# scale-lab/MTLoRA

Hardware: AMD Instinct MI355X
Metric: images/sec (train step) Swin-T/448 r=64 4-task (higher is better)
Workload: dtype bf16; 1 GPU; BASELINE configs[1]: Swin-T 448, 4 tasks (semseg,normals,sal,human_parts), r_shared=64 r_task=4 scale4; train step (fwd+loss+bwd+clip+AdamW), dropout .05, drop_path .2; per_gpu_batch=32, global_batch=32, img_size=448, parallelism=dp1, trainable_params=8344634, allreduce_bytes=0

## Files before the change

mtlora_amd/csrc/linear.hip:

```cpp
#include <string.h>
#include <algorithm>
#include <atomic>
#include <type_traits>

#include "common.h"
#include "internal.h"
#include "hid_params.h"
#include "nt.h"
#include "stream.h"
#include "dense.h"
#include "pq.h"
#include "tn.h"

namespace {

static Segs make_segs(const mtlora_linear_desc* d) {
    Segs s;
    s.n = 1 + d->T;
    int off = 0;
    for (int o = 0; o < s.n; ++o) {
        int r = (o == 0) ? d->r_s : d->r_t[o - 1];
        s.r[o] = r;
        s.rp[o] = (int)mtl_round_up(r, 8);
        s.off[o] = off;
        off += s.rp[o];
    }
    for (int o = s.n; o < MAXO; ++o) s.r[o] = s.rp[o] = s.off[o] = 0;
    s.used = off;
    s.R = (int)mtl_round_up(off, 16);
    return s;
}

static CtxLayout ctx_layout(const mtlora_linear_desc* d, const Segs& s) {
    const int es = mtl_elem_size(d->dtype);
    CtxLayout L;
    int64_t o = 0;
    auto take = [&](int64_t bytes) {
        int64_t at = o;
        o += mtl_round_up(bytes, 256);
        return at;
    };
    L.a_cat = take((int64_t)s.R * d->K * es);
    L.b_cat = take((int64_t)d->N * s.R * es);
    L.at_cat = take((int64_t)d->K * s.R * es);
    L.bt_cat = take((int64_t)s.R * d->N * es);
    L.alpha = take((int64_t)s.R * 4);
    L.a_proj = take((int64_t)s.R * d->K * es);
    L.bt_proj = take((int64_t)s.R * d->N * es);
    L.b_frag = take(mtl_round_up(d->N, 32) * mtl_round_up(s.R, 32) * es);
    L.at_frag = take(mtl_round_up(d->K, 32) * mtl_round_up(s.R, 32) * es);
    L.pack_total = o;
    if (d->packed) o = 0;
    L.p = take(d->M * s.R * es);
    L.total = o;
    return L;
}

static int check_desc(const mtlora_linear_desc* d) {
    if (!d) return MTLORA_ERR_NULL;
    if (d->dtype != MTLORA_F32 && d->dtype != MTLORA_BF16 && d->dtype != MTLORA_F16) return MTLORA_ERR_DTYPE;
    if (d->M < 0 || d->K <= 0 || d->N <= 0 || d->T < 0 || d->T > MTLORA_MAX_TASKS || d->r_s < 0)
        return MTLORA_ERR_SHAPE;
    if (d->M >= ((int64_t)1 << 31)) return MTLORA_ERR_SHAPE;
    const int vec = d->dtype == MTLORA_F32 ? 4 : 8;
    if (d->K % vec || d->N % vec) return MTLORA_ERR_ALIGN;
    for (int t = 0; t < d->T; ++t)
        if (d->r_t[t] <= 0) return MTLORA_ERR_SHAPE;
    if (d->mode != 0 && d->mode != 1) return MTLORA_ERR_UNSUPPORTED;
    if (d->bwd_phase < 0 || d->bwd_phase > 2) return MTLORA_ERR_UNSUPPORTED;
    if (d->sel_stream < 0 || d->sel_stream > 1 || d->sel_dense < 0 || d->sel_dense > 4 || d->sel_tn < 0 || d->sel_tn > 2 || d->sel_projk < 0 ||
        d->sel_projk > 3 || d->max_cu < 0)
        return MTLORA_ERR_UNSUPPORTED;
    if (d->dropout_p < 0.f || d->dropout_p >= 1.f) return MTLORA_ERR_SHAPE;
    return MTLORA_OK;
}

static bool misaligned(const void* p) { return ((uintptr_t)p & 15u) != 0; }

struct Tune {
    int sp, ntd, tn, projk, max_cu;
};
static Tune make_tune(const mtlora_linear_desc* d) {
    auto tri = [](int v) { return v == 1 ? 0 : (v == 2 ? 2 : 1); };
    Tune t;
    t.sp = d->sel_stream == 1 ? 0 : 1;
    t.ntd = d->sel_dense >= 3 ? d->sel_dense : tri(d->sel_dense);
    t.tn = tri(d->sel_tn);
    t.projk = d->sel_projk == 3 ? 3 : tri(d->sel_projk);
    t.max_cu = d->max_cu > 0 ? d->max_cu : 0;
    return t;
}
constexpr int MTL_MAX_DEV = 64;
static int cur_dev() {
    int dev = 0;
    (void)hipGetDevice(&dev);
    return dev >= 0 && dev < MTL_MAX_DEV ? dev : 0;
}
static int dev_num_cu() {
    static std::atomic<int> cache[MTL_MAX_DEV];
    const int dev = cur_dev();
    int cu = cache[dev].load(std::memory_order_relaxed);
    if (cu == 0) {
        cu = 256;
        (void)hipDeviceGetAttribute(&cu, hipDeviceAttributeMultiprocessorCount, dev);
        if (cu <= 0) cu = 256;
        cache[dev].store(cu, std::memory_order_relaxed);
    }
    return cu;
}
static int num_cu(const Tune& tu) {
    const int cu = dev_num_cu();
    return tu.max_cu > 0 && tu.max_cu < cu ? tu.max_cu : cu;
}
static bool raise_lds(std::atomic<unsigned long long>& done, const void* fn, int bytes) {
    const int dev = cur_dev();
    if ((done.load(std::memory_order_relaxed) >> dev) & 1ull) return true;
    if (hipFuncSetAttribute(fn, hipFuncAttributeMaxDynamicSharedMemorySize, bytes) != hipSuccess) {
        (void)hipGetLastError();
        return false;
    }
    done.fetch_or(1ull << dev, std::memory_order_relaxed);
    return true;
}
#define MTL_RAISE_LDS(KERNEL, BYTES)                                        \
    do {                                                                    \
        static std::atomic<unsigned long long> done__{0};                   \
        (void)raise_lds(done__, (const void*)(KERNEL), (int)(BYTES));       \
    } while (0)

static bool nte_prefer(int64_t tiles, int ksteps, int64_t cus) {
    const double eff_d = (double)tiles / (double)(mtl_ceil_div(tiles, cus) * cus);
    return (ksteps >= 4 && ksteps <= 12 && tiles * 2 >= 3 * cus) || (ksteps >= 6 && eff_d < 0.7 && tiles >= cus);
}

static NlParams make_nl(const NtParams& P, int64_t mt, int64_t nt, bool dense) {
    NlParams q;
    q.act = reinterpret_cast<const bf16*>(P.act[0]);
    q.wgt = reinterpret_cast<const bf16*>(P.wgt);
    q.L = reinterpret_cast<const bf16*>(P.L);
    q.Rm = reinterpret_cast<const bf16*>(P.Rm);
    q.out = reinterpret_cast<bf16*>(P.out[0].ptr);
    q.act2 = reinterpret_cast<bf16*>(P.out[0].act);
    q.gate = dense ? reinterpret_cast<const bf16*>(P.out[0].gate) : nullptr;
    q.bias = P.bias;
    q.alpha = P.alpha;
    q.ld_act = P.ld_act;
    q.ld_wgt = P.ld_wgt;
    q.ldL = P.ldL;
    q.ldR = P.ldR;
    q.ld_out = P.ld_out;
    q.M = (int)P.M;
    q.n_rows = P.n_rows;
    q.K = P.act[0] ? P.K : 0;
    q.seg_lo = P.L ? P.out[0].seg_lo : 0;
    q.seg_hi = P.L ? P.out[0].seg_hi : 0;
    q.n_tiles = (int)nt;
    q.nt_magic = (uint32_t)(((uint64_t)1 << 32) / (uint64_t)nt) + 1u;
    const uint32_t nwg = (uint32_t)(mt * nt);
    q.q8 = nwg / 8u;
    q.r8 = nwg % 8u;
    q.act_mask = dense ? 0 : P.act_mask;
    q.use_base = P.out[0].use_base;
    q.drop = P.drop;
    return q;
}

template <typename F>
static void nl_dispatch(const NlParams& q, bool ml0, F&& go) {
    using Y = std::true_type;
// ... 162 lines not shown
    MtlProfScope prof(kind, alg_bytes, s, s8d, flops);
    const size_t lds = (size_t)q.n_blk_total * 32 * q.K * 2 + (size_t)SP_WAVES * ns * 32 * ch * 2;
    const int per_cu = lds * 2 <= (size_t)SP_LDS_MAX ? 2 : 1;
    int64_t wgs = mtl_ceil_div(q.n_items, SP_WAVES);
    if (wgs > (int64_t)num_cu(tu) * per_cu) wgs = (int64_t)num_cu(tu) * per_cu;
#define MTL_SP_PROJ(CHV, NSV)                                                                              \
    do {                                                                                                   \
        MTL_RAISE_LDS((k_sp_proj<T, CHV, NSV>), SP_LDS_MAX);                                               \
        hipLaunchKernelGGL((k_sp_proj<T, CHV, NSV>), dim3((unsigned)wgs), dim3(64 * SP_WAVES), lds, s, q); \
    } while (0)
    if constexpr (sizeof(T) == 2) {
        if (ch == 96) {
            if (ns == 3) MTL_SP_PROJ(96, 3);
            else if (ns == 2) MTL_SP_PROJ(96, 2);
            else MTL_SP_PROJ(96, 1);
        } else {
            if (ns == 3) MTL_SP_PROJ(64, 3);
            else if (ns == 2) MTL_SP_PROJ(64, 2);
            else MTL_SP_PROJ(64, 1);
        }
    }
#undef MTL_SP_PROJ
}

template <typename T>
static int pq_plan(const Tune& tu, const SpProjParams& q, PqParams& pq) {
    if (sizeof(T) != 2 || tu.sp == 0 || tu.projk == 0 || tu.projk == 2 || q.M <= 0 || q.n_src < 1 || q.n_src > MAXO) return 0;
    if (q.Rw % 8 != 0 || q.K % 8 != 0 || q.K < 32 || (q.ld_out % 8) != 0) return 0;
    if ((((uintptr_t)q.wproj | (uintptr_t)q.out) & 15u) != 0) return 0;
    if (q.M >= ((int64_t)1 << 31) - 256 || q.M * q.ld_out * 2 >= ((int64_t)1 << 32) - 64) return 0;
    int wmax = 0;
    for (int s = 0; s < q.n_src; ++s) {
        const SpSrc& ss = q.src[s];
        if (((uintptr_t)ss.act & 15u) != 0 || ss.col_lo % 8 != 0 || ss.col_hi % 8 != 0 || ss.col_hi <= ss.col_lo || ss.col_hi > q.Rw) return 0;
        if (ss.col_hi - ss.col_lo > 1024) return 0;
        pq.src[s].act = ss.act;
        pq.src[s].col_lo = ss.col_lo;
        pq.src[s].col_hi = ss.col_hi;
        pq.src[s].mask = ss.mask;
        pq.src[s].pad_ = 0;
        wmax = ss.col_hi - ss.col_lo > wmax ? ss.col_hi - ss.col_lo : wmax;
    }
    pq.n_src = q.n_src;
    pq.wproj = q.wproj;
    pq.out = q.out;
    pq.ld_out = q.ld_out;
    pq.M = (int)q.M;
    pq.K = q.K;
    pq.R = q.Rw;
    pq.drop = q.drop;
    const int64_t per_row_tile = (int64_t)q.n_src * mtl_ceil_div(wmax, wmax > 64 ? 128 : 64);
    return mtl_ceil_div(q.M, 64) * per_row_tile * 4 <= (int64_t)num_cu(tu) * 5 ? 1 : 2;
}
static bool pq_one_round(const Tune& tu, const PqParams& pq, int mb) {
    return pq.n_src == 1 && mtl_ceil_div(pq.M, 64 * mb) * 4 <= (int64_t)num_cu(tu) * 5;
}
template <typename T>
static void launch_pq(const PqParams& pq, int mb, hipStream_t s, int kind, double alg_bytes, double s8d, double flops) {
    int wmax = 0, any_mask = 0;
    for (int i = 0; i < pq.n_src; ++i) {
        wmax = pq.src[i].col_hi - pq.src[i].col_lo > wmax ? pq.src[i].col_hi - pq.src[i].col_lo : wmax;
        any_mask |= pq.src[i].mask;
    }
    mtl_prof_tag("pq M%d K%d R%d src%d w%d mb%d mask%d", pq.M, pq.K, pq.R, pq.n_src, wmax, mb, any_mask);
    MtlProfScope prof(kind, alg_bytes, s, s8d, flops);
    const bool wide = wmax > 64;
    const dim3 grid((unsigned)mtl_ceil_div(pq.M, 64 * mb), (unsigned)mtl_ceil_div(wmax, wide ? 128 : 64), (unsigned)pq.n_src);
#define MTL_PQ(WMV, NBV, NSTV, KSV)                                                                               \
    do {                                                                                                          \
        constexpr size_t lds = (size_t)NSTV * (32 * WMV + 32 * NBV) * 64;                                         \
        MTL_RAISE_LDS((k_pq<T, WMV, NBV, NSTV, KSV>), SP_LDS_MAX);                                                \
        hipLaunchKernelGGL((k_pq<T, WMV, NBV, NSTV, KSV>), grid, dim3(256), lds, s, pq);                          \
    } while (0)
    if constexpr (sizeof(T) == 2) {
        const bool ksp = any_mask != 0 && pq.drop.enabled();
        if (mb == 1 && wide && ksp) MTL_PQ(2, 4, 6, true);
        else if (mb == 1 && wide) MTL_PQ(2, 4, 6, false);
        else if (mb == 1 && ksp) MTL_PQ(2, 2, 8, true);
        else if (mb == 1) MTL_PQ(2, 2, 8, false);
        else if (wide) MTL_PQ(4, 4, 5, false);
        else MTL_PQ(4, 2, 6, false);
    }
#undef MTL_PQ
}

template <typename T>
static bool sp_projk_plan(const Tune& tu, SpProjParams& q, int& ch) {
    if (sizeof(T) != 2 || tu.sp == 0 || q.M <= 0 || q.n_src <= 0) return false;
    const int mode = tu.projk;
    if (mode == 0) return false;
    ch = q.K % 96 == 0 ? 96 : (q.K % 64 == 0 ? 64 : 0);
    if (ch == 0 || q.M >= ((int64_t)1 << 31) - 64) return false;
    q.n_blk_total = (q.Rw + 31) / 32;
    for (int s = 0; s < q.n_src; ++s) {
        if (q.src[s].n_blk > SP_MAXB || q.src[s].n_blk <= 0) return false;
        if (((uintptr_t)q.src[s].act & 15u) != 0) return false;
    }
    if ((q.ld_out % 8) != 0 || ((uintptr_t)q.out & 15u) != 0 || ((uintptr_t)q.wproj & 15u) != 0) return false;
    if (q.M * q.ld_out * 2 >= ((int64_t)1 << 32) - 64) return false;
    q.n_slabs = (int)mtl_ceil_div(q.M, 32);
    q.n_items = q.n_slabs * q.n_src;
    return mode == 2 || (mode == 1 && (int64_t)q.n_items <= (int64_t)num_cu(tu) && q.K / ch >= SP_WAVES);
}
template <typename T>
static void launch_sp_projk(const Tune& tu, const SpProjParams& q, int ch, hipStream_t s, int kind, double alg_bytes, double s8d, double flops) {
    mtl_prof_tag("sp_projk M%lld K%d R%d src%d ch%d", (long long)q.M, q.K, q.Rw, q.n_src, ch);
    MtlProfScope prof(kind, alg_bytes, s, s8d, flops);
    int64_t wgs = q.n_items;
    if (wgs > (int64_t)num_cu(tu)) wgs = num_cu(tu);
#define MTL_SP_PROJK(CHV, NSLV)                                                                                   \
    do {                                                                                                          \
        constexpr size_t slots = (size_t)SP_WAVES * NSLV * 32 * CHV * 2, red = (size_t)SP_WAVES * SP_MAXB * 4096; \
        constexpr size_t lds = slots > red ? slots : red;                                                         \
        MTL_RAISE_LDS((k_sp_projk<T, CHV, NSLV>), SP_LDS_MAX);                                                    \
        hipLaunchKernelGGL((k_sp_projk<T, CHV, NSLV>), dim3((unsigned)wgs), dim3(64 * SP_WAVES), lds, s, q);      \
    } while (0)
    if constexpr (sizeof(T) == 2) {
        if (ch == 96)
            MTL_SP_PROJK(96, 3);
        else
            MTL_SP_PROJK(64, 4);
    }
#undef MTL_SP_PROJK
}

template <typename T>
static void launch_sp_projsum(const Tune& tu, const SpProjParams& q, int ch, int ns, T* gsum, hipStream_t s, int kind, double alg_bytes,
                              double s8d, double flops) {
    mtl_prof_tag("sp_projsum M%lld K%d R%d src%d ch%d ns%d", (long long)q.M, q.K, q.Rw, q.n_src, ch, ns);
    MtlProfScope prof(kind, alg_bytes, s, s8d, flops);
    const size_t lds = (size_t)q.n_blk_total * 32 * q.K * 2 + (size_t)SP_WAVES * ns * 32 * ch * 2;
    int64_t wgs = mtl_ceil_div(q.n_slabs, SP_WAVES);
    if (wgs > (int64_t)num_cu(tu)) wgs = num_cu(tu);
#define MTL_SP_PS(CHV, NSV)                                                                                         \
    do {                                                                                                            \
        MTL_RAISE_LDS((k_sp_projsum<T, CHV, NSV>), SP_LDS_MAX);                                                     \
        hipLaunchKernelGGL((k_sp_projsum<T, CHV, NSV>), dim3((unsigned)wgs), dim3(64 * SP_WAVES), lds, s, q, gsum); \
    } while (0)
    if constexpr (sizeof(T) == 2) {
        if (ch == 96) {
            if (ns >= 2) MTL_SP_PS(96, 2);
            else MTL_SP_PS(96, 1);
        } else {
            if (ns >= 2) MTL_SP_PS(64, 2);
            else MTL_SP_PS(64, 1);
        }
    }
#undef MTL_SP_PS
}

struct SpXresPlan {
    int ch, nkc, nrb;
    bool stg;
    unsigned grid;
    size_t lds;
};
static unsigned sp_lin_grid(const Tune& tu, int parts, int n_slabs, int& xsh) {
    const int64_t cu = num_cu(tu);
    const int64_t by_slabs = mtl_ceil_div(n_slabs, SP_WAVES);
    if (cu >= 8 * (int64_t)parts) {
        xsh = 3;
        int64_t g8 = mtl_ceil_div(by_slabs, 8);
        const int64_t g8_max = cu / (8 * parts);
        if (g8 > g8_max) g8 = g8_max;
        return (unsigned)(8 * parts * g8);
    }
// ... 399 lines not shown
        q.drop = dc;
        if (j.one_panel) {
            q.act[0] = src[0].act;
            q.act_mask = src[0].mask;
            q.n_rows = sg.R;
        } else {
            for (int i = 0; i < n_src; ++i) {
                q.zact[i] = src[i].act;
                q.zrow0[i] = src[i].col_lo;
                q.zrows[i] = src[i].col_hi - src[i].col_lo;
                q.zmask[i] = src[i].mask;
            }
            q.nz = n_src;
        }
        launch_nt<T>(tu, q, s, j.kind, j.alg_bytes, j.s8d, j.flops);
    }
}

static double rank_sum(const Segs& sg, const void* const* live = nullptr) {
    double rsum = 0.0;
    for (int o = 0; o < sg.n; ++o)
        if (!live || (sg.rp[o] > 0 && live[o])) rsum += sg.r[o];
    return rsum;
}
static double fused_bytes(const mtlora_linear_desc* d, int es) { return (double)es * d->M * (d->K + (double)d->N); }
static double fused_flops(const mtlora_linear_desc* d, const Segs& sg) {
    return 2.0 * d->M * (double)d->K * d->N + 2.0 * d->M * (double)sg.r[0] * (d->K + d->N);
}

template <typename T>
static bool fwd_one_pass(const mtlora_linear_desc* d, const Tune& tu, const Segs& sg, const CtxLayout& L, const unsigned char* pk, const void* x,
                         const void* W, const float* bias, void* y_s, void* a_s, T* Pm, const DropoutCfg& dc, hipStream_t s) {
    SpLinParams q = {};
    q.act = x;
    q.w = W;
    q.proj = pk + L.a_proj;
    q.expand = pk + L.b_frag;
    q.bias = bias;
    q.out = y_s;
    q.out2 = a_s;
    q.pout = Pm;
    q.ld_out = d->N;
    q.ldp = sg.R;
    q.M = d->M;
    q.n_cols = (int)d->N;
    q.R = sg.R;
    q.mask_act = 1;
    q.mask_lr = 0;
    q.drop = dc;
    SpXresPlan pl;
    const double b8d = fused_bytes(d, (int)sizeof(T)), fl = fused_flops(d, sg);
    if (sp_xres_plan<T>(tu, q, (int)d->K, pl)) {
        launch_sp_xres<T>(q, pl, a_s != nullptr, s, PK_NT_FWD_MAIN, b8d + (a_s ? (double)sizeof(T) * d->M * d->N : 0.0), b8d, fl);
        return true;
    }
    SpAresPlan pa;
    q.estep = q.estep2 = 0;
    if (a_s == nullptr && sp_ares_plan<T>(tu, q, (int)d->K, pa)) {
        launch_sp_ares<T>(q, pa, s, PK_NT_FWD_MAIN, b8d, b8d, fl);
        return true;
    }
    return false;
}

template <typename T>
static int fwd_impl(const mtlora_linear_desc* d, const void* x, const void* const* x_t, const void* W,
                    const float* bias, const float* A_s, const float* B_s, const float* const* A_t,
                    const float* const* B_t, void* y_s, void* const* y_t, void* ctx, hipStream_t s, void* a_s = nullptr,
                    void* const* a_t = nullptr) {
    const Segs sg = make_segs(d);
    const Tune tu = make_tune(d);
    const CtxLayout L = ctx_layout(d, sg);
    unsigned char* c = reinterpret_cast<unsigned char*>(ctx);
    unsigned char* pk = d->packed ? const_cast<unsigned char*>(reinterpret_cast<const unsigned char*>(d->packed)) : c;
    T* a_cat = reinterpret_cast<T*>(pk + L.a_cat);
    T* b_cat = reinterpret_cast<T*>(pk + L.b_cat);
    float* alpha = reinterpret_cast<float*>(pk + L.alpha);
    T* Pm = reinterpret_cast<T*>(c + L.p);
    const DropoutCfg dc = mtl_make_dropout(d->dropout_p, d->seed, d->seed_offset);

    if (sg.R > 0) {
        if (!d->packed) launch_pack<T>(d, sg, L, pk, A_s, B_s, A_t, B_t, s);
        if (d->T == 0 && d->mode == 0 && fwd_one_pass<T>(d, tu, sg, L, pk, x, W, bias, y_s, a_s, Pm, dc, s)) return MTLORA_OK;

        const bool own = d->T > 0 && d->has_x_tasks;
        ProjSrc src[MAXO];
        int n_src = 0;
        if (!own) src[n_src++] = ProjSrc{x, 0, sg.used, 1};
        for (int o = 0; own && o < sg.n; ++o) {
            if (sg.rp[o] == 0) continue;
            if (o > 0 && (d->hid & MTLORA_HID_P_GIVEN)) continue;
            src[n_src++] = ProjSrc{o == 0 ? x : x_t[o - 1], sg.off[o], sg.off[o] + sg.rp[o], o == 0 ? 1 : 0};
        }
        const double xb = (double)sizeof(T) * ((d->has_x_tasks && !(d->hid & MTLORA_HID_P_GIVEN)) ? d->T : 0) * d->M * d->K;
        ProjJob<T> j = {};
        j.wproj = pk + L.a_proj;
        j.wcat = a_cat;
        j.alpha = alpha;
        j.out = Pm;
        j.M = d->M;
        j.K = (int)d->K;
        j.one_panel = !own;
        j.kind = PK_NT_FWD_P;
        j.alg_bytes = j.s8d = xb;
        j.flops = 2.0 * d->M * d->K * rank_sum(sg);
        launch_proj<T>(tu, sg, dc, s, src, n_src, j);
    }

    NtParams m = {};
    m.act[0] = x;
    m.n_act = 1;
    m.ld_act = d->K;
    m.wgt = W;
    m.ld_wgt = d->K;
    m.M = d->M;
    m.n_rows = (int)d->N;
    m.K = (int)d->K;
    m.bias = bias;
    m.L = Pm;
    m.ldL = sg.R;
    m.Rm = b_cat;
    m.ldR = sg.R;
    m.ld_out = d->N;
    m.drop = dc;
    m.n_out = 1 + d->T;
    for (int o = 0; o < sg.n; ++o) {
        NtOut& O = m.out[o];
        O.ptr = (o == 0) ? y_s : y_t[o - 1];
        O.seg_lo = sg.off[o];
        O.seg_hi = sg.off[o] + sg.rp[o];
        O.use_base = 1;
        O.mask_lr = 0;
        O.fold = (o == 0 && d->mode == 1 && d->T > 0) ? 1 : 0;
        O.act = (o == 0) ? a_s : (a_t ? a_t[o - 1] : nullptr);
    }
    if (d->hid & MTLORA_HID_FWD_BASE) {
        m.n_out = 2;
        NtOut& O = m.out[1];
        O.ptr = const_cast<void*>(d->hid_ptr);
        O.seg_lo = O.seg_hi = 0;
        O.use_base = 1;
        O.mask_lr = 0;
        O.fold = 0;
        O.act = nullptr;
    }
    int n_actout = 0;
    for (int o = 0; o < m.n_out; ++o) n_actout += m.out[o].act ? 1 : 0;
    const double b8d = (double)sizeof(T) * d->M * (d->K + (double)(1 + d->T) * d->N);
    const double fl = 2.0 * d->M * d->K * d->N + 2.0 * d->M * d->N * rank_sum(sg);
    const bool plain = sg.R == 0;
    launch_nt<T>(tu, m, s, plain ? PK_NT_PLAIN_FWD : PK_NT_FWD_MAIN, b8d + (double)sizeof(T) * d->M * (double)n_actout * d->N,
                 plain ? 0.0 : b8d, fl);
    return MTLORA_OK;
}

constexpr int64_t TN_TARGET_CTAS = 512;
struct BwdScratch {
    int64_t q, g, part, total;
    int nsplit;
    int64_t rows_per_split;
};
static BwdScratch bwd_scratch(const mtlora_linear_desc* d, const Segs& sg) {
    const int es = mtl_elem_size(d->dtype);
    BwdScratch S;
    int64_t o = 0;
    auto take = [&](int64_t bytes) {
// ... 65 lines not shown
};

template <typename T>
static void bwd_grad_sum(Bwd<T>& b) {
    const mtlora_linear_desc* d = b.d;
    const Segs& sg = b.sg;
    const bool v2 = d->mode == 1 && d->T > 0;
    b.presum = b.n_dy > 1 && b.dx && mtl_ceil_div(d->K, TILE) >= 3;
    b.have_g = false;
    b.q_done = false;
    if constexpr (sizeof(T) == 2) {
        if (d->T >= 1 && d->mode == 0 && b.do_dx && b.dx && b.n_dy == 1 + d->T && sg.rp[0] > 0 && sg.rp[0] <= 64) {
            ProjSrc src[MAXO];
            bool ok = true;
            for (int o = 0; o < sg.n; ++o) {
                if (sg.rp[o] == 0 || (o > 0 && sg.rp[o] > 32)) ok = false;
                src[o] = ProjSrc{b.dy[o], sg.off[o], sg.off[o] + sg.rp[o], 0};
            }
            SpProjParams sp = make_sp_proj(src, sg.n, b.pk + b.L.bt_proj, b.Qm, sg, d->M, (int)d->N, b.dc);
            for (int o = 1; o < sg.n; ++o)
                if (sp.src[o].n_blk != 1) ok = false;
            if (ok && sp.src[sp.n_src - 1].blk_lo - sp.src[1].blk_lo + 1 > SP_PS_MAXT) ok = false;
            int ch = 0;
            const int ns = ok ? sp_proj_plan<T>(b.tu, sp, ch) : 0;
            if (ns > 0 && d->M * d->N * 2 < ((int64_t)1 << 32) - 64) {
                launch_sp_projsum<T>(b.tu, sp, ch, ns, b.Gm, b.s, PK_NT_BWD_Q, 0.0, 0.0, 2.0 * d->M * d->N * rank_sum(sg));
                b.q_done = true;
                b.presum = true;
                b.have_g = true;
            }
        }
    }
    if ((v2 || b.presum) && b.n_dy > 1) b.have_g = true;
    if (b.have_g && b.do_dx && !b.q_done) {
        SumParams sp;
        sp.n = b.n_dy;
        for (int i = 0; i < b.n_dy; ++i) sp.src[i] = b.dy_all[i];
        sp.nvec = d->M * d->N / ET<T>::VEC;
        int64_t blocks = mtl_ceil_div(sp.nvec, 256);
        if (blocks > 4096) blocks = 4096;
        if (blocks > 0) {
            MtlProfScope prof(PK_SUM, (double)sizeof(T) * d->M * d->N * (b.n_dy + 1), b.s);
            hipLaunchKernelGGL(k_sum<T>, dim3((unsigned)blocks), dim3(256), 0, b.s, sp, b.Gm);
        }
    }
    const void* dy_shared = b.dy[0];
    if (v2 && b.n_dy > 0) dy_shared = b.have_g ? (const void*)b.Gm : b.dy_all[0];
    for (int o = 0; o < sg.n; ++o) b.dyo[o] = (o == 0) ? dy_shared : b.dy[o];
}

template <typename T>
static bool bwd_one_pass(Bwd<T>& b) {
    const mtlora_linear_desc* d = b.d;
    const Segs& sg = b.sg;
    if (!(d->T == 0 && d->mode == 0 && b.do_dx && b.dx && b.dyo[0] && sg.R > 0)) return false;
    SpLinParams q = {};
    q.act = b.dyo[0];
    q.w = b.Wt;
    q.proj = b.pk + b.L.bt_proj;
    q.expand = b.pk + b.L.at_frag;
    q.out = b.dx;
    q.pout = b.Qm;
    q.ld_out = d->K;
    q.ldp = sg.R;
    q.M = d->M;
    q.n_cols = (int)d->K;
    q.R = sg.R;
    q.mask_act = 0;
    q.mask_lr = 1;
    q.drop = b.dc;
    const double b8d = fused_bytes(d, (int)sizeof(T)), fl = fused_flops(d, sg);
    SpAresPlan pl;
    if (!b.gate_s && sp_ares_plan<T>(b.tu, q, (int)d->N, pl)) {
        launch_sp_ares<T>(q, pl, b.s, PK_NT_BWD_DX, b8d, b8d, fl);
        return true;
    }
    SpXresPlan px;
    q.gate = b.gate_s;
    if (sp_xres_plan<T>(b.tu, q, (int)d->N, px)) {
        launch_sp_xres<T>(q, px, false, b.s, PK_NT_BWD_DX, b8d + (b.gate_s ? (double)sizeof(T) * d->M * d->K : 0.0), b8d, fl, b.gate_s != nullptr);
        return true;
    }
    return false;
}

template <typename T>
static void bwd_q(Bwd<T>& b) {
    const mtlora_linear_desc* d = b.d;
    const Segs& sg = b.sg;
    if (!(sg.R > 0 && b.do_dx && !b.q_done)) return;
    bool any_missing = false;
    ProjSrc src[MAXO];
    int n_src = 0;
    for (int o = 0; o < sg.n; ++o) {
        if (sg.rp[o] == 0) continue;
        if (!b.dyo[o]) {
            any_missing = true;
            continue;
        }
        src[n_src++] = ProjSrc{b.dyo[o], sg.off[o], sg.off[o] + sg.rp[o], 0};
    }
    if (any_missing && !b.hid_q) mtl_zero_async(b.Qm, (size_t)(d->M * sg.R * sizeof(T)), b.s);
    if (n_src > 0) {
        ProjJob<T> j = {};
        j.wproj = b.pk + b.L.bt_proj;
        j.wcat = b.bt_cat;
        j.alpha = b.alpha;
        j.out = b.Qm;
        j.M = d->M;
        j.K = (int)d->N;
        j.kind = PK_NT_BWD_Q;
        j.flops = 2.0 * d->M * d->N * rank_sum(sg, b.dyo);
        launch_proj<T>(b.tu, sg, b.dc, b.s, src, n_src, j);
    }
}

template <typename T>
static void bwd_dx(Bwd<T>& b) {
    const mtlora_linear_desc* d = b.d;
    const Segs& sg = b.sg;
    const Tune& tu = b.tu;
    hipStream_t s = b.s;
    void* const* dx_t = b.dx_t;
    const void* const* gate_t = b.gate_t;
    if (!b.do_dx) return;
    NtParams m = {};
    RankOutParams rank_out = {};
    int rank_out_rp = 8;
    bool rank_out_gated = false;
    if (b.presum && b.have_g) {
        m.n_act = 1;
        m.act[0] = b.Gm;
    } else {
        m.n_act = b.n_dy;
        for (int i = 0; i < b.n_dy; ++i) m.act[i] = b.dy_all[i];
    }
    if (b.hid_q && d->hid_ptr) {
        m.n_act = 1;
        m.act[0] = d->hid_ptr;
    }
    m.ld_act = d->N;
    m.wgt = b.Wt;
    m.ld_wgt = d->N;
    m.M = d->M;
    m.n_rows = (int)d->K;
    m.K = (b.n_dy > 0 || (b.hid_q && d->hid_ptr)) ? (int)d->N : 0;
    m.L = b.Qm;
    m.ldL = sg.R;
    m.Rm = b.at_cat;
    m.ldR = sg.R;
    m.ld_out = d->K;
    m.drop = b.dc;
    m.n_out = 1;
    NtOut& O = m.out[0];
    O.ptr = b.dx;
    O.use_base = 1;
    O.mask_lr = 1;
    O.gate = b.gate_s;
    if (d->T > 0 && d->has_x_tasks) {
        O.seg_lo = sg.off[0];
        O.seg_hi = sg.off[0] + sg.rp[0];
        if constexpr (sizeof(T) == 2) {
            bool ok = tu.sp != 0 && dx_t != nullptr && d->K % 8 == 0 && d->K / 8 <= 256 && d->M > 0;
            int rpm = 0, gates = 0, outs = 0;
            for (int t = 0; t < d->T; ++t) {
                if (!dx_t || !dx_t[t]) continue;
// ... 142 lines not shown
        if (!b.dyo[o]) dBo = nullptr;
        if (dBo) add_tn_problem(tp, pp, S.nsplit, b.Pm, sg.R, sg.off[o], sg.rp[o], b.dyo[o], (int)d->N, 0, dBo, sg.r[o], sg.r[o], 1);
        const bool own_x = (o > 0 && d->has_x_tasks);
        if (dAo) add_tn_problem(tp, pp, S.nsplit, b.Qm, sg.R, sg.off[o], sg.rp[o], own_x ? b.x_t[o - 1] : b.x, (int)d->K, own_x ? 0 : 1, dAo, sg.r[o], (int)d->K, 0);
    }
    int max_tiles = 0;
    double fl = 0.0;
    for (int i = 0; i < tp.n_prob; ++i) {
        max_tiles = std::max(max_tiles, tp.p[i].tiles_a * tp.p[i].tiles_b);
        fl += 2.0 * d->M * (double)tp.p[i].out_a * tp.p[i].out_b;
    }
    const double xb = (double)sizeof(T) * d->M * (double)(1 + (d->has_x_tasks ? d->T : 0)) * d->K;
    if constexpr (sizeof(T) == 2) {
        const int nb = (tu.sp != 0 && tu.tn != 0) ? sp_tn_nb(d) : 0;
        SpTnParams q = {};
        bool ok = sp_tn_table(tp, nb, q);
        if (ok) {
            const int mode = tu.tn;
            q.n_prob = tp.n_prob;
            q.G = sp_tn_groups(tu, q.n_pp, d->M);
            ok = q.n_pp <= SP_TN_WGS && q.G < 65536 && (mode == 2 || (mode == 1 && mtl_ceil_div(d->M, 32) >= (int64_t)8 * q.G * SP_WAVES));
            if (ok) {
                SpTnParams probe = q;
                ok = sp_tn_map(probe) != 0;
                q.G = probe.G;
            }
        }
        if (ok) {
            q.M = d->M;
            q.part = b.part;
            q.drop = b.dc;
            char tag[96];
            snprintf(tag, sizeof(tag), "M%lld K%lld N%lld T%d", (long long)d->M, (long long)d->K, (long long)d->N, d->T);
            launch_sp_tn<T>(q, nb, s, xb, fl, tag);
            return;
        }
    }
    if (tp.n_prob > 0 && d->M > 0) {
        {
            mtl_prof_tag("M%lld K%lld N%lld T%d np%d ns%d tiles%d", (long long)d->M, (long long)d->K, (long long)d->N, d->T, tp.n_prob,
                         S.nsplit, max_tiles);
            MtlProfScope prof(PK_TN, xb, s, xb, fl);
            hipLaunchKernelGGL(k_tn<T>, dim3((unsigned)S.nsplit, (unsigned)max_tiles, (unsigned)tp.n_prob),
                               dim3(256), 0, s, tp);
        }
        MtlProfScope prof(PK_REDUCE, 0.0, s);
        hipLaunchKernelGGL(k_tn_reduce, dim3(TN_TILE / 1024, (unsigned)max_tiles, (unsigned)tp.n_prob), dim3(256 * TN_RG), 0, s, tp);
    }
}

template <typename T>
static int bwd_impl(const mtlora_linear_desc* d, const void* x, const void* const* x_t, const void* Wt,
                    const void* dy_s, const void* const* dy_t, const void* ctx, void* dx, void* const* dx_t,
                    float* dA_s, float* dB_s, float* const* dA_t, float* const* dB_t, void* scratch, hipStream_t s,
                    const void* gate_s = nullptr, const void* const* gate_t = nullptr) {
    Bwd<T> b = {};
    b.d = d;
    b.sg = make_segs(d);
    b.tu = make_tune(d);
    b.L = ctx_layout(d, b.sg);
    b.S = bwd_scratch(d, b.sg);
    b.s = s;
    b.dc = mtl_make_dropout(d->dropout_p, d->seed, d->seed_offset);
    const unsigned char* c = reinterpret_cast<const unsigned char*>(ctx);
    unsigned char* sc = reinterpret_cast<unsigned char*>(scratch);
    b.pk = d->packed ? reinterpret_cast<const unsigned char*>(d->packed) : c;
    b.at_cat = reinterpret_cast<const T*>(b.pk + b.L.at_cat), b.bt_cat = reinterpret_cast<const T*>(b.pk + b.L.bt_cat);
    b.alpha = reinterpret_cast<const float*>(b.pk + b.L.alpha);
    b.Pm = reinterpret_cast<const T*>(c + b.L.p);
    b.Qm = reinterpret_cast<T*>(sc + b.S.q), b.Gm = reinterpret_cast<T*>(sc + b.S.g);
    b.part = reinterpret_cast<float*>(sc + b.S.part);
    b.x = x, b.x_t = x_t, b.Wt = Wt;
    b.dx = dx, b.dx_t = dx_t;
    b.dA_s = dA_s, b.dB_s = dB_s, b.dA_t = dA_t, b.dB_t = dB_t;
    b.gate_s = gate_s, b.gate_t = gate_t;
    b.do_dx = d->bwd_phase != 2;
    b.hid_q = (d->hid & MTLORA_HID_Q_GIVEN) != 0;
    b.dy[0] = dy_s;
    for (int t = 0; t < d->T; ++t) b.dy[t + 1] = dy_t ? dy_t[t] : nullptr;
    for (int o = 0; o < b.sg.n; ++o)
        if (b.dy[o]) b.dy_all[b.n_dy++] = b.dy[o];

    bwd_grad_sum(b);
    if (!bwd_one_pass(b)) {
        bwd_q(b);
        bwd_dx(b);
    }
    if (d->bwd_phase != 1) bwd_factors(b);
    return MTLORA_OK;
}

struct HidPlan {
    int tg, rr, nthr, nw, groups, n_wg;
};
static int hid_check(const mtlora_linear_desc* d1, const mtlora_linear_desc* d2) {
    int st = check_desc(d1);
    if (st != MTLORA_OK) return st;
    st = check_desc(d2);
    if (st != MTLORA_OK) return st;
    if (d1->dtype == MTLORA_F32 || d1->dtype != d2->dtype) return MTLORA_ERR_UNSUPPORTED;
    if (d1->M != d2->M || d1->N != d2->K || d1->T != d2->T || d1->T < 1) return MTLORA_ERR_UNSUPPORTED;
    if (d1->mode != 0 || d2->mode != 0 || !d1->has_x_tasks || !d2->has_x_tasks) return MTLORA_ERR_UNSUPPORTED;
    if (d1->N % 128 != 0 || d1->M <= 0) return MTLORA_ERR_UNSUPPORTED;
    int rmax = 0;
    for (int t = 0; t < d1->T; ++t) {
        if (d1->r_t[t] < 1 || d1->r_t[t] > 8 || d2->r_t[t] < 1 || d2->r_t[t] > 8) return MTLORA_ERR_UNSUPPORTED;
        rmax = std::max(rmax, std::max(d1->r_t[t], d2->r_t[t]));
    }
    const bool chunked = d1->sel_stream != 1 && rmax <= 4;
    if (d1->N > 2048 && !chunked) return MTLORA_ERR_UNSUPPORTED;
    return MTLORA_OK;
}
static HidPlan hid_plan(const mtlora_linear_desc* d1, const mtlora_linear_desc* d2) {
    HidPlan pl;
    int rmax = 0;
    for (int t = 0; t < d1->T; ++t) rmax = std::max(rmax, std::max(d1->r_t[t], d2->r_t[t]));
    pl.rr = rmax <= 4 ? 4 : 8;
    pl.nthr = (int)(d1->N / 2);
    pl.nw = pl.nthr / 64;
    const int cap = pl.nthr <= 512 ? 16 : 8;
    pl.tg = std::max(1, cap / pl.rr);
    if (pl.nthr > 768 && pl.rr == 8) pl.tg = 1;
    pl.groups = (d1->T + pl.tg - 1) / pl.tg;
    const Tune tu = make_tune(d1);
    const int wg_per_cu = std::max(1, (8 + pl.nw - 1) / pl.nw);
    const int64_t nblk = (d1->M + HID_RB - 1) / HID_RB;
    pl.n_wg = (int)std::min<int64_t>(nblk, (int64_t)num_cu(tu) * wg_per_cu);
    return pl;
}
static int64_t hid_part_bytes(const mtlora_linear_desc* d1, const HidPlan& pl) {
    const Tune tu = make_tune(d1);
    const int64_t slots = std::max<int64_t>((int64_t)pl.n_wg * pl.tg, (int64_t)num_cu(tu) * HID_TG);
    return slots * 2 * pl.rr * d1->N * 4 + 256;
}

static void hid_launch_valu(int dtype, bool bwd, const HidPlan& pl, const HidParams& q, hipStream_t s) {
    HidLaunch L = {};
    L.kind = bwd ? 1 : 0;
    L.dtype = dtype;
    L.tg = pl.tg;
    L.rr = pl.rr;
    L.nthr = pl.nthr;
    L.n_wg = pl.n_wg;
    mtli_hid_launch(&L, &q, s);
}
struct HidDPlan {
    bool on;
    int hc, n_chunk, n_wg, groups;
    size_t lds_f, lds_b;
    int64_t rowpart_bytes;
};
static HidDPlan hid_d_plan(const mtlora_linear_desc* d1, const HidPlan& pl, bool bwd) {
    HidDPlan dp = {};
    const Tune tu = make_tune(d1);
    const int H = (int)d1->N;
    dp.hc = hid_d_chunk(H, bwd);
    dp.on = tu.sp != 0 && pl.rr == 4 && dp.hc != 0;
    if (!dp.on) return dp;
    dp.n_chunk = H / dp.hc;
    dp.groups = (d1->T + HID_TG - 1) / HID_TG;
    dp.lds_f = hid_d_lds_bytes(dp.hc, false);
    dp.lds_b = hid_d_lds_bytes(dp.hc, true);
    const int64_t nblk = (d1->M + 31) / 32;
    const int per_cu = std::max(1, std::min((int)((size_t)(150 * 1024) / (bwd ? dp.lds_b : dp.lds_f)), (bwd ? 12 : 16) / (dp.hc / 32)));
    dp.n_wg = (int)std::min<int64_t>(nblk, std::max<int64_t>(1, (int64_t)num_cu(tu) * per_cu / dp.n_chunk));
    dp.rowpart_bytes = (int64_t)dp.n_chunk * d1->M * 16 * 4 + 256;
    return dp;
// ... 510 lines not shown
```

Baseline: 1146 images/sec.

## Add fused panel kernel for LoRA linear with 384-wide output, fwd and bwd-dx

Adds a persistent 512-thread kernel that computes the dense GEMM, the LoRA down-projection, the rank expansion, bias and dropout in a single pass over a 128-row tile covering the full 384-column output, with a 4-stage LDS DMA ring. It is used for single-task (T==0) forward and backward-dx when N or K equals 384. With the default selector it runs only when the block count sits between half and all of the CUs and K is 384, 1152 or 1536. The goal is to cut separate launches and activation re-reads. The cost is high register and LDS pressure and limited occupancy.

```diff
diff --git a/mtlora_amd/csrc/linear.hip b/mtlora_amd/csrc/linear.hip
--- a/mtlora_amd/csrc/linear.hip
+++ b/mtlora_amd/csrc/linear.hip
@@ -10,6 +10,7 @@
 #include "stream.h"
 #include "dense.h"
 #include "pq.h"
+#include "panel.h"
 #include "tn.h"
 
 namespace {
@@ -68,7 +69,7 @@
         if (d->r_t[t] <= 0) return MTLORA_ERR_SHAPE;
     if (d->mode != 0 && d->mode != 1) return MTLORA_ERR_UNSUPPORTED;
     if (d->bwd_phase < 0 || d->bwd_phase > 2) return MTLORA_ERR_UNSUPPORTED;
-    if (d->sel_stream < 0 || d->sel_stream > 1 || d->sel_dense < 0 || d->sel_dense > 4 || d->sel_tn < 0 || d->sel_tn > 2 || d->sel_projk < 0 ||
+    if (d->sel_stream < 0 || d->sel_stream > 1 || d->sel_dense < 0 || d->sel_dense > 7 || d->sel_dense == 5 || d->sel_tn < 0 || d->sel_tn > 2 || d->sel_projk < 0 ||
         d->sel_projk > 3 || d->max_cu < 0)
         return MTLORA_ERR_UNSUPPORTED;
     if (d->dropout_p < 0.f || d->dropout_p >= 1.f) return MTLORA_ERR_SHAPE;
@@ -78,13 +79,14 @@
 static bool misaligned(const void* p) { return ((uintptr_t)p & 15u) != 0; }
 
 struct Tune {
-    int sp, ntd, tn, projk, max_cu;
+    int sp, ntd, tn, projk, panel, max_cu;
 };
 static Tune make_tune(const mtlora_linear_desc* d) {
     auto tri = [](int v) { return v == 1 ? 0 : (v == 2 ? 2 : 1); };
     Tune t;
     t.sp = d->sel_stream == 1 ? 0 : 1;
-    t.ntd = d->sel_dense >= 3 ? d->sel_dense : tri(d->sel_dense);
+    t.ntd = d->sel_dense >= 6 ? 1 : (d->sel_dense >= 3 ? d->sel_dense : tri(d->sel_dense));
+    t.panel = d->sel_dense == 6 ? 2 : (d->sel_dense == 0 ? 1 : 0);
     t.tn = tri(d->sel_tn);
     t.projk = d->sel_projk == 3 ? 3 : tri(d->sel_projk);
     t.max_cu = d->max_cu > 0 ? d->max_cu : 0;
@@ -413,6 +415,40 @@
         else MTL_PQ(4, 2, 6, false);
     }
 #undef MTL_PQ
+}
+
+static bool panel_prefer(int64_t M, int Kred, int64_t cus) {
+    const int64_t blocks = mtl_ceil_div(M, PN_TM);
+    return (Kred == 384 || Kred == 1152 || Kred == 1536) && blocks <= cus && 2 * blocks > cus;
+}
+template <typename T>
+static bool panel_plan(const Tune& tu, const Segs& sg, int64_t M, int Kred, int64_t Nout, const PnParams& q) {
+    if (sizeof(T) != 2 || tu.sp == 0 || tu.panel == 0 || M <= 0 || Nout != PN_NOUT || Kred < 384 || Kred % PN_KE != 0) return false;
+    if (sg.R <= 0 || sg.R > PN_RMAX || sg.used <= 0) return false;
+    if (M >= ((int64_t)1 << 31) - 256 || M * PN_NOUT * 2 >= ((int64_t)1 << 32) - 64 || M * Kred * 2 >= ((int64_t)1 << 32) - 64) return false;
+    const void* ptrs[] = {q.act, q.w, q.proj, q.expand, q.bias, q.out, q.pout};
+    for (const void* pp : ptrs)
+        if (((uintptr_t)pp & 15u) != 0) return false;
+    if (!q.act || !q.w || !q.out || !q.pout) return false;
+    return tu.panel == 2 || panel_prefer(M, Kred, num_cu(tu));
+}
+template <typename T>
+static void launch_panel(const Tune& tu, const PnParams& q, bool mlr, hipStream_t s, int kind, double alg_bytes, double s8d, double flops) {
+    mtl_prof_tag("pnr M%d K%d N%d R%d mlr%d", q.M, q.K, PN_NOUT, q.R, mlr ? 1 : 0);
+    MtlProfScope prof(kind, alg_bytes, s, s8d, flops);
+    int64_t wgs = mtl_ceil_div(q.M, PN_TM);
+    if (wgs > (int64_t)num_cu(tu)) wgs = num_cu(tu);
+#define MTL_PNR(MAV, MLV)                                                                                  \
+    do {                                                                                                   \
+        MTL_RAISE_LDS((k_pnr<T, MAV, MLV>), SP_LDS_MAX);                                                   \
+        hipLaunchKernelGGL((k_pnr<T, MAV, MLV>), dim3((unsigned)wgs), dim3(512), (size_t)PN_LDS, s, q);    \
+    } while (0)
+    if constexpr (sizeof(T) == 2) {
+        if (!q.drop.enabled()) MTL_PNR(false, false);
+        else if (mlr) MTL_PNR(false, true);
+        else MTL_PNR(true, false);
+    }
+#undef MTL_PNR
 }
 
 template <typename T>
@@ -978,6 +1014,26 @@
     if (sg.R > 0) {
         if (!d->packed) launch_pack<T>(d, sg, L, pk, A_s, B_s, A_t, B_t, s);
         if (d->T == 0 && d->mode == 0 && fwd_one_pass<T>(d, tu, sg, L, pk, x, W, bias, y_s, a_s, Pm, dc, s)) return MTLORA_OK;
+        if (d->T == 0 && d->mode == 0 && d->hid == 0 && a_s == nullptr) {
+            PnParams q = {};
+            q.act = x;
+            q.w = W;
+            q.proj = pk + L.a_proj;
+            q.expand = b_cat;
+            q.bias = bias;
+            q.out = y_s;
+            q.pout = Pm;
+            q.M = (int)d->M;
+            q.K = (int)d->K;
+            q.R = sg.R;
+            q.used = sg.used;
+            q.drop = dc;
+            if (panel_plan<T>(tu, sg, d->M, (int)d->K, d->N, q)) {
+                const double b8d = fused_bytes(d, (int)sizeof(T));
+                launch_panel<T>(tu, q, false, s, PK_NT_FWD_MAIN, b8d, b8d, 2.0 * d->M * d->K * d->N + 2.0 * d->M * d->N * rank_sum(sg));
+                return MTLORA_OK;
+            }
+        }
 
         const bool own = d->T > 0 && d->has_x_tasks;
         ProjSrc src[MAXO];
@@ -1209,6 +1265,29 @@
         return true;
     }
     return false;
+}
+
+template <typename T>
+static bool bwd_panel(Bwd<T>& b) {
+    const mtlora_linear_desc* d = b.d;
+    const Segs& sg = b.sg;
+    if (!(d->T == 0 && d->mode == 0 && d->hid == 0 && b.do_dx && b.dx && b.dyo[0] && b.n_dy == 1 && !b.gate_s && sg.R > 0)) return false;
+    PnParams q = {};
+    q.act = b.dyo[0];
+    q.w = b.Wt;
+    q.proj = b.pk + b.L.bt_proj;
+    q.expand = b.at_cat;
+    q.out = b.dx;
+    q.pout = b.Qm;
+    q.M = (int)d->M;
+    q.K = (int)d->N;
+    q.R = sg.R;
+    q.used = sg.used;
+    q.drop = b.dc;
+    if (!panel_plan<T>(b.tu, sg, d->M, (int)d->N, d->K, q)) return false;
+    const double b8d = fused_bytes(d, (int)sizeof(T));
+    launch_panel<T>(b.tu, q, true, b.s, PK_NT_BWD_DX, b8d, b8d, 2.0 * d->M * d->N * d->K + 2.0 * d->M * d->K * rank_sum(sg, b.dyo));
+    return true;
 }
 
 template <typename T>
@@ -1517,7 +1596,7 @@
         if (b.dy[o]) b.dy_all[b.n_dy++] = b.dy[o];
 
     bwd_grad_sum(b);
-    if (!bwd_one_pass(b)) {
+    if (!bwd_one_pass(b) && !bwd_panel(b)) {
         bwd_q(b);
         bwd_dx(b);
     }
diff --git a/mtlora_amd/csrc/panel.h b/mtlora_amd/csrc/panel.h
--- /dev/null
+++ b/mtlora_amd/csrc/panel.h
@@ -0,0 +1,247 @@
+#pragma once
+
+#include "nt.h"
+#include "stream.h"
+
+namespace {
+
+constexpr int PN_TM = 128, PN_NOUT = 384, PN_RMAX = 64, PN_KE = 32;
+constexpr int PN_ROWS = PN_NOUT + PN_RMAX + PN_TM;
+constexpr int PN_STAGE = PN_ROWS * 64;
+constexpr int PN_NST = 4;
+constexpr int PN_LDS = PN_NST * PN_STAGE;
+constexpr int PN_NDMA = PN_ROWS / 16;
+constexpr int PN_PRS = PN_RMAX * 2 + 16;
+constexpr int PN_ORS = 96 * 2 + 8;
+constexpr int PN_RED = 0, PN_PIMG = 4 * 2 * 16 * 256, PN_OIMG = PN_PIMG + PN_TM * PN_PRS;
+static_assert(PN_OIMG + 8 * 32 * PN_ORS <= PN_LDS, "the ring holds the tail images");
+
+struct PnParams {
+    const void* act;
+    const void* w;
+    const void* proj;
+    const void* expand;
+    const float* bias;
+    void* out;
+    void* pout;
+    int M, K, R, used;
+    DropoutCfg drop;
+};
+
+template <typename T, bool MASKED, bool MLR>
+__global__ __launch_bounds__(512) void k_pnr(const PnParams P) {
+    extern __shared__ __attribute__((aligned(16))) unsigned char smem[];
+    const int tid = threadIdx.x, lane = tid & 63, wave = __builtin_amdgcn_readfirstlane(tid >> 6);
+    const int wm = wave >> 2, wn = wave & 3, h = lane >> 5, rl = lane & 31;
+    const int pks = wn & 1, psm = wn >> 1;
+    const int M = P.M, K = P.K, R = P.R, used = P.used;
+    const unsigned char* const act = reinterpret_cast<const unsigned char*>(P.act);
+    const unsigned char* const wgt = reinterpret_cast<const unsigned char*>(P.w);
+    const unsigned char* const prj = reinterpret_cast<const unsigned char*>(P.proj);
+    const T* const expand = reinterpret_cast<const T*>(P.expand);
+    const float* const bias = P.bias;
+    DropoutCfg drop = P.drop;
+    mtl_dropout_resolve(drop);
+    const bool masked = drop.thr16 != 0;
+    const int total = K / PN_KE;
+    const __amdgpu_buffer_rsrc_t orsrc = sp_rsrc(P.out, (int64_t)M * PN_NOUT * 2);
+    const __amdgpu_buffer_rsrc_t prsrc = sp_rsrc(P.pout, (int64_t)M * R * 2);
+
+    const int dpw = wave < 4 ? 5 : 4;
+    const int lrow = lane >> 2;
+    const int q8 = ((lane & 3) ^ ((lrow >> 2) & 3)) * 8;
+    const uint32_t wsrc = (uint32_t)(((16 * wave + lrow) * K + q8) * 2), wstep = (uint32_t)(128 * K * 2);
+    const int pr = 16 * wave + lrow;
+    const uint32_t psrc = (uint32_t)(((pr < R ? pr : R - 1) * K + q8) * 2);
+    const int arow = wave < 4 ? 64 + 16 * wave + lrow : 16 * (wave - 4) + lrow;
+    auto wait_stage = [&](int n) __attribute__((always_inline)) {
+        if (n == 0) SP_WAIT_VM(0);
+        else if (dpw == 5) { if (n == 1) SP_WAIT_VM(5); else SP_WAIT_VM(10); }
+        else { if (n == 1) SP_WAIT_VM(4); else SP_WAIT_VM(8); }
+    };
+
+    int co[2];
+#pragma unroll
+    for (int ks = 0; ks < 2; ++ks) co[ks] = (((2 * ks + h) ^ ((rl >> 2) & 3)) << 4) + rl * 64;
+    const int w_off = (wn * 96) * 64, p_off = PN_NOUT * 64, a_off = (PN_NOUT + PN_RMAX + wm * 64) * 64;
+
+    const int n_blk = (M + PN_TM - 1) / PN_TM;
+    for (int blk = blockIdx.x; blk < n_blk; blk += gridDim.x) {
+        const int m0 = blk * PN_TM;
+        const uint32_t asrc = ((uint32_t)(m0 + arow < M ? m0 + arow : M - 1) * (uint32_t)K + (uint32_t)q8) * 2u;
+        auto issue = [&](int i) __attribute__((always_inline)) {
+            const uint32_t k0 = (uint32_t)(i * PN_KE * 2);
+            unsigned char* dst = smem + (i % PN_NST) * PN_STAGE + wave * 1024;
+#pragma unroll
+            for (int t = 0; t < 3; ++t) sp_dma16(wgt + (wsrc + t * wstep + k0), dst + t * 8192);
+            if (wave < 4) {
+                sp_dma16(prj + (psrc + k0), dst + 3 * 8192);
+                sp_dma16(act + (asrc + k0), dst + 4 * 8192);
+            } else {
+                sp_dma16(act + (asrc + k0), dst + 3 * 8192);
+            }
+        };
+#pragma unroll
+        for (int i = 0; i < PN_NST - 1; ++i)
+            if (i < total) issue(i);
+
+        f32x16 acc[2][3], accp[2];
+#pragma unroll
+        for (int e = 0; e < 16; ++e) {
+#pragma unroll
+            for (int sm = 0; sm < 2; ++sm)
+#pragma unroll
+                for (int b = 0; b < 3; ++b) acc[sm][b][e] = 0.f;
+            accp[0][e] = accp[1][e] = 0.f;
+        }
+        const uint32_t rhp = mtl_dropout_rowhash(drop, 0u, (uint32_t)(m0 + wm * 64 + psm * 32 + rl));
+
+        for (int i = 0; i < total; ++i) {
+            const int rest = total - 1 - i;
+            wait_stage(rest < PN_NST - 2 ? rest : PN_NST - 2);
+            asm volatile("" ::: "memory");
+            SP_WAIT_LGKM0();
+            __builtin_amdgcn_s_barrier();
+            asm volatile("" ::: "memory");
+            if (i + PN_NST - 1 < total) issue(i + PN_NST - 1);
+            const unsigned char* st = smem + (i % PN_NST) * PN_STAGE;
+#pragma unroll
+            for (int ks = 0; ks < 2; ++ks) {
+                u32x4 fa[2], fw[3];
+#pragma unroll
+                for (int sm = 0; sm < 2; ++sm) fa[sm] = *reinterpret_cast<const u32x4*>(st + a_off + sm * 32 * 64 + co[ks]);
+#pragma unroll
+                for (int b = 0; b < 3; ++b) fw[b] = *reinterpret_cast<const u32x4*>(st + w_off + b * 32 * 64 + co[ks]);
+                if (ks == pks) {
+                    u32x4 fp[2], fm = psm ? fa[1] : fa[0];
+#pragma unroll
+                    for (int rb = 0; rb < 2; ++rb) fp[rb] = *reinterpret_cast<const u32x4*>(st + p_off + rb * 32 * 64 + co[ks]);
+                    if constexpr (MASKED) {
+                        if (masked) VOps<T>::drop(fm, drop, rhp, (uint32_t)(i * PN_KE + ks * 16 + 8 * h));
+                    }
+#pragma unroll
+                    for (int rb = 0; rb < 2; ++rb) sp_mma1<T>(fp[rb], fm, accp[rb]);
+                }
+#pragma unroll
+                for (int sm = 0; sm < 2; ++sm)
+#pragma unroll
+                    for (int b = 0; b < 3; ++b) sp_mma1<T>(fw[b], fa[sm], acc[sm][b]);
+            }
+        }
+        __syncthreads();
+
+        {
+            float* red = reinterpret_cast<float*>(smem + PN_RED) + (wm * 2 + psm) * (2 * 16 * 64);
+            if (pks == 1) {
+#pragma unroll
+                for (int rb = 0; rb < 2; ++rb)
+#pragma unroll
+                    for (int e = 0; e < 16; ++e) red[(rb * 16 + e) * 64 + lane] = accp[rb][e];
+            }
+            __syncthreads();
+            if (pks == 0) {
+                unsigned char* prow = smem + PN_PIMG + (wm * 64 + psm * 32 + rl) * PN_PRS;
+#pragma unroll
+                for (int rb = 0; rb < 2; ++rb)
+#pragma unroll
+                    for (int q = 0; q < 4; ++q) {
+                        float v[4];
+#pragma unroll
+                        for (int e = 0; e < 4; ++e) v[e] = accp[rb][q * 4 + e] + red[(rb * 16 + q * 4 + e) * 64 + lane];
+                        const int r = rb * 32 + 8 * q + 4 * h;
+                        u32x2 pk = {mtl_pk2<T>(v[0], v[1]), mtl_pk2<T>(v[2], v[3])};
+                        if (r >= used) pk = u32x2{0u, 0u};
+                        *reinterpret_cast<u32x2*>(prow + r * 2) = pk;
+                    }
+            }
+            __syncthreads();
+#pragma unroll
+            for (int it = 0; it < 2; ++it) {
+                const int idx = it * 512 + tid, ml = idx >> 3, c = idx & 7;
+                const u32x4 v = *reinterpret_cast<const u32x4*>(smem + PN_PIMG + ml * PN_PRS + c * 16);
+                const int m = m0 + ml, r = c * 8;
+                sp_bstore(v, prsrc, (m < M && r < used) ? (uint32_t)m * (uint32_t)(R * 2) + (uint32_t)r * 2u : 0xFFFFFFFFu);
+            }
+        }
+
+#pragma unroll
+        for (int b = 0; b < 3; ++b) {
+            __builtin_amdgcn_sched_barrier(0);
+            const int nb = wn * 96 + b * 32;
+            u32x4 fe[4];
+#pragma unroll
+            for (int ks = 0; ks < 4; ++ks) {
+                const int r = ks * 16 + 8 * h;
+                fe[ks] = u32x4{0u, 0u, 0u, 0u};
+                if (r < used) fe[ks] = *reinterpret_cast<const u32x4*>(expand + (int64_t)(nb + rl) * R + r);
+            }
+#pragma unroll
+            for (int sm = 0; sm < 2; ++sm) {
+                f32x16 lr;
+#pragma unroll
+                for (int e = 0; e < 16; ++e) lr[e] = 0.f;
+                const unsigned char* prow = smem + PN_PIMG + (wm * 64 + sm * 32 + rl) * PN_PRS + 16 * h;
+#pragma unroll
+                for (int ks = 0; ks < 4; ++ks) {
+                    const u32x4 fq = *reinterpret_cast<const u32x4*>(prow + ks * 32);
+                    sp_mma1<T>(fe[ks], fq, lr);
+                }
+                if constexpr (MLR) {
+                    if (masked) {
+                        const uint32_t rh = mtl_dropout_rowhash(drop, 0u, (uint32_t)(m0 + wm * 64 + sm * 32 + rl));
+#pragma unroll
+                        for (int q = 0; q < 4; ++q) {
+                            const int n = nb + 8 * q + 4 * h;
+                            const uint32_t h0 = mtl_dropout_pairbits(drop, rh, (uint32_t)n);
+                            const uint32_t h1 = mtl_dropout_pairbits(drop, rh, (uint32_t)(n + 2));
+                            if ((h0 & 0xFFFFu) < drop.thr16) lr[q * 4 + 0] = 0.f;
+                            if ((h0 >> 16) < drop.thr16) lr[q * 4 + 1] = 0.f;
+                            if ((h1 & 0xFFFFu) < drop.thr16) lr[q * 4 + 2] = 0.f;
+                            if ((h1 >> 16) < drop.thr16) lr[q * 4 + 3] = 0.f;
+                        }
+                    }
+                }
+#pragma unroll
+                for (int e = 0; e < 16; ++e) acc[sm][b][e] += lr[e];
+            }
+            if (bias) {
+#pragma unroll
+                for (int q = 0; q < 4; ++q) {
+                    const f32x4 bi = *reinterpret_cast<const f32x4*>(bias + nb + 8 * q + 4 * h);
+#pragma unroll
+                    for (int sm = 0; sm < 2; ++sm)
+#pragma unroll
+                        for (int e = 0; e < 4; ++e) acc[sm][b][q * 4 + e] += bi[e];
+                }
+            }
+        }
+
+        unsigned char* img = smem + PN_OIMG + wave * (32 * PN_ORS);
+#pragma unroll
+        for (int sm = 0; sm < 2; ++sm) {
+            __builtin_amdgcn_sched_barrier(0);
+#pragma unroll
+            for (int b = 0; b < 3; ++b)
+#pragma unroll
+                for (int q = 0; q < 4; ++q) {
+                    const int nl = b * 32 + 8 * q + 4 * h;
+                    u32x2 pk = {mtl_pk2<T>(acc[sm][b][q * 4], acc[sm][b][q * 4 + 1]), mtl_pk2<T>(acc[sm][b][q * 4 + 2], acc[sm][b][q * 4 + 3])};
+                    *reinterpret_cast<u32x2*>(img + rl * PN_ORS + nl * 2) = pk;
+                }
+            SP_WAIT_LGKM0();
+            __builtin_amdgcn_wave_barrier();
+#pragma unroll
+            for (int it = 0; it < 6; ++it) {
+                const int idx = it * 64 + lane, ml = idx / 12, c16 = idx - ml * 12;
+                const int m = m0 + wm * 64 + sm * 32 + ml, n = wn * 96 + c16 * 8;
+                const u32x4 v = *reinterpret_cast<const u32x4*>(img + ml * PN_ORS + c16 * 16);
+                sp_bstore(v, orsrc, m < M ? (uint32_t)m * (uint32_t)(PN_NOUT * 2) + (uint32_t)n * 2u : 0xFFFFFFFFu);
+            }
+            SP_WAIT_LGKM0();
+            __builtin_amdgcn_wave_barrier();
+        }
+        __syncthreads();
+    }
+}
+
+}
```

Result: slower. 1107 images/sec (-3.4%).
